# witalis3/UHSDR

Hardware: AMD Instinct MI355X
Metric: Msamples/s through full SSB-RX chain (node); % of HBM-roofline per GPU (higher is better)
Workload: dtype f32; 1 GPU; C2: 4096 ch x 256-frame blocks, SSB-USB P48 chain, f32; channels_per_gpu=4096, frames_per_call=256, parallelism=channel-sharded x1, no data-path collective, outputs=f32 audio, pipelined=True, handoff=persistent, precision=exact, schedule=split_pipe

## Files before the change

uhsdr_amd/csrc/uhsdr_dsp.h:

```cpp
#ifndef UHSDR_DSP_H
#define UHSDR_DSP_H

#include <hip/hip_runtime.h>
#include <stdint.h>
#include "uhsdr_internal.h"

#define BLK UHSDR_IQ_BLOCK_SIZE
#define IQ_BIT_SCALE_DOWN 0.0000152587890625f

typedef float vf4 __attribute__((ext_vector_type(4)));

template <int V, int N>
__device__ __forceinline__ void lds_vec(const float* p, float (&w)[N], int j)
{
    if (V == 4)
    {
        const float4 v = *(const float4*)p;
        w[j] = v.x; w[j + 1] = v.y; w[j + 2] = v.z; w[j + 3] = v.w;
    }
    else
    {
        const float2 v = *(const float2*)p;
        w[j] = v.x; w[j + 1] = v.y;
    }
// ... 107 lines not shown
        }
        else
        {
#pragma unroll
            for (int q = 0; q < 8; ++q) cc[q] = c[8 * ch + q];
        }
        v2f nw[8];
#pragma unroll
        for (int q = 0; q < 8; q += 2)
        {
            const vf4 v = *(const vf4*)(win + (16 + PB) * ch + pwin_off<PB>(WA + q));
            nw[q] = v.xy; nw[q + 1] = v.zw;
        }
#pragma unroll
        for (int kk = 0; kk < 8; ++kk)
        {
#pragma unroll
            for (int r = 0; r < R; ++r) acc[r] = fir_mac<F>(acc[r], w[r * M + kk], cc[kk]);
        }
#pragma unroll
        for (int j = 0; j < WA - 8; ++j) w[j] = w[j + 8];
#pragma unroll
        for (int q = 0; q < 8; ++q) w[WA - 8 + q] = nw[q];
    }
#pragma unroll
    for (int kk = 0; kk < TR; ++kk)
    {
        const v2f ck = TP ? cn[kk] : c[8 * NCH + kk];
#pragma unroll
        for (int r = 0; r < R; ++r) acc[r] = fir_mac<F>(acc[r], w[r * M + kk], ck);
    }
}

constexpr int FRONT_TAIL = 8;

__device__ __forceinline__ float to_vgpr(float x)
{
    float r;
    asm volatile("v_mov_b32 %0, %1" : "=v"(r) : "s"(x));
    return r;
}
template <int N>
__device__ __forceinline__ void to_vgpr(float (&x)[N])
{
#pragma unroll
    for (int i = 0; i < N; ++i) x[i] = to_vgpr(x[i]);
}

__device__ __forceinline__ void wave_sync()
{
    __builtin_amdgcn_fence(__ATOMIC_RELEASE, "wavefront");
    __builtin_amdgcn_wave_barrier();
    __builtin_amdgcn_fence(__ATOMIC_ACQUIRE, "wavefront");
}

__device__ __forceinline__ void lds_barrier()
{
    asm volatile("s_waitcnt lgkmcnt(0)" ::: "memory");
    __builtin_amdgcn_s_barrier();
    asm volatile("" ::: "memory");
}

constexpr int FRONT_WAVE = 64;
#define FRONT_WAVE_L 64

__host__ __device__ constexpr int hist_stride(int T) { return (T - 1 + 3) & ~3; }
__host__ __device__ constexpr int hist_q(int T) { return (hist_stride(T) / 4 + 7) / 8; }


template <int T, int HQM>
__device__ __forceinline__ void front_load_row(const float* row, int cl, int b, int nb, vf4 (&buf)[HQM])
{
    constexpr int hs4 = hist_stride(T) / 4, HQ = hist_q(T);
    const vf4* h = (const vf4*)(row + (size_t)cl * (hs4 * 4));
#pragma unroll
    for (int i = 0; i < HQ; ++i)
    {
        const int q = b + nb * i;
        buf[i] = h[q < hs4 ? q : hs4 - 1];
    }
}

template <int T, int HQM>
__device__ __forceinline__ void front_fill(float* W, float* row, int c, bool act, bool live, int b, int nb,
                                           const vf4 (&buf)[HQM], const float* vals, int NV)
{
// ... 234 lines not shown
        if (((T - 1 + b * NV) & 3) == 0 && (NV & 3) == 0)
            for (int j = 0; j < NV; j += 4) *(vf4*)(d + j) = vf4{ vals[j], vals[j + 1], vals[j + 2], vals[j + 3] };
        else if (((T - 1 + b * NV) & 1) == 0 && (NV & 1) == 0)
            for (int j = 0; j < NV; j += 2) *(v2f*)(d + j) = v2f{ vals[j], vals[j + 1] };
        else
            for (int j = 0; j < NV; ++j) d[j] = vals[j];
    }
}

__host__ __device__ inline void front_lane(int l, int nb, int S, int& g, int& b)
{
    const int cpw = 64 / nb, K = 64 / S, cpg = S / 4;
    if ((nb & (nb - 1)) || nb < K || cpw < cpg)
    {
        g = l / nb;
        b = l % nb;
        return;
    }
    const int h = l & 31;
    int k, j;
    if (h < 4) { k = 0; j = h; }
    else if (h < 12) { k = 1; j = h - 4; }
    else if (h < 16) { k = 0; j = h - 8; }
    else if (h < 20) { k = 1; j = h - 8; }
    else if (h < 28) { k = 0; j = h - 12; }
    else { k = 1; j = h - 16; }
    k += (l >> 5) * 2;
    const int pr = k * cpg + j / K;
    g = pr % cpw;
    b = (pr / cpw) * K + j % K;
}

template <int S>
__device__ __forceinline__ float lattice_step(float x, float (&g)[S > 0 ? S : 1], const float* k, const float* v)
{
    float fcurr = x, fnext = 0.0f, acc = 0.0f;
    float gn[S > 0 ? S : 1];
#pragma unroll
    for (int i = 0; i < S; ++i)
    {
        const float gcurr = g[i];
        fnext = fcurr - (k[i] * gcurr);
        const float gnext = (fnext * k[i]) + gcurr;
        acc += (gnext * v[i]);
        gn[i] = gnext;
        fcurr = fnext;
    }
    acc += (fnext * v[S]);
#pragma unroll
    for (int i = 0; i + 1 < S; ++i) g[i] = gn[i + 1];
    if (S > 0) g[S - 1] = fnext;
    return acc;
}

template <int S, int PAR>
__device__ __forceinline__ float lattice_step_pk(float x, float (&g)[S > 0 ? S : 1], const float* k, const float* v)
{
    if constexpr (S < 3) return lattice_step<S>(x, g, k, v);
    else
    {
        float gn[S], q[S];
        float f = x;
        int i = 0;
        if (PAR)
        {
            f = f - (k[0] * g[0]);
// ... 211 lines not shown
```

uhsdr_amd/csrc/uhsdr_rx.hip:

```cpp

#include <hip/hip_runtime.h>
#include <hip/hip_ext.h>
#include <stdint.h>
#include <string.h>
#include <stdlib.h>
#include <math.h>
#include <chrono>
#include "uhsdr_internal.h"
#include "uhsdr_libm.h"
#include "uhsdr_log10f_fast.h"
#include "uhsdr_dsp.h"

#define BACK_CH 64
constexpr int CNT_PITCH = 32;

struct FrontArgs
{
    const uhsdr_rx_plan* plan;
    const int2* iq;
    float* hist1;
    float* hist2;
    const uint16_t* lanemap;
    const uint16_t* lanemap2;
    int nb, cpw;
    float* teta;
    int* tp;
    unsigned* clip;
    const float* osc_in;
    float* osc_out;
    float* adec;
    float* adec_q;
    const float* taps2a;
    const float* taps2b;
    int C, N, ld, ldd;
    int lw;
    int comb;
    float* fm_prev;
    unsigned* gcnt;
};

enum { FRONT_COMB_USB = 0,
       FRONT_COMB_LSB = 1,
       FRONT_COMB_I = 2,
       FRONT_COMB_SSB_ST = 3,
       FRONT_COMB_IQ_ST = 4 };

template <int R>
__device__ __forceinline__ void front_comb_block(int comb, const v2f (&h)[R], float (&o)[R])
{
    if (comb == FRONT_COMB_I)
    {
#pragma unroll
        for (int r = 0; r < R; ++r) o[r] = h[r].x;
    }
    else if (comb == FRONT_COMB_LSB)
    {
#pragma unroll
        for (int r = 0; r < R; ++r) o[r] = h[r].x - h[r].y;
    }
    else
    {
#pragma unroll
        for (int r = 0; r < R; ++r) o[r] = h[r].x + h[r].y;
    }
}
__device__ __forceinline__ v2f front_comb2(int comb, v2f h)
{
    return comb == FRONT_COMB_SSB_ST ? v2f{ h.x + h.y, h.x - h.y } : h;
}

struct InputStage
// ... 90 lines not shown
    }
    if (!s.iq_auto)
    {
        if (s.gi != 1.0f || s.gq != 1.0f)
        {
#pragma unroll
            for (int j = 0; j < R; ++j) { xi[j] = xi[j] * s.gi; xq[j] = xq[j] * s.gq; }
        }
        if (s.ph < 0)
        {
#pragma unroll
            for (int j = 0; j < R; ++j) { const float e3 = xi[j] * s.ph; xq[j] = xq[j] + e3; }
        }
        else if (s.ph > 0)
        {
#pragma unroll
            for (int j = 0; j < R; ++j) { const float e3 = xq[j] * s.ph; xi[j] = xi[j] + e3; }
        }
    }
    else
    {
        const int bb = n0 / BLK;
        const float f1 = m1[bb], f2 = m2[bb];
#pragma unroll
        for (int j = 0; j < R; ++j) { xq[j] += f1 * xi[j]; xi[j] = xi[j] * f2; }
    }
    if (s.shift)
    {
        if (s.shift_up) freq_shift_block<R>(xi, xq, s.shift, osc, n0);
        else freq_shift_block<R>(xq, xi, s.shift, osc, n0);
    }
}

template <int T1, int T2, int M, bool DECIM_FIRST, int R, bool F, bool ST, typename Sink>
__device__ __forceinline__ void front_body(const FrontArgs& a, const int grp, float* smem, Sink&& sink)
{
    const uhsdr_rx_plan* __restrict__ P = a.plan;
    const int N = a.N, C = a.C;
    const int lane = threadIdx.x & (FRONT_WAVE - 1);
    const int nb = a.nb;
    const int CPW = a.cpw;
    const unsigned lm = a.lanemap[lane];
    const int g = (int)(lm >> 8), b = (int)(lm & 0xffu);
    const bool act = g < CPW;
    const int gs = act ? g : 0;
    const int nblk32 = N / BLK;
    constexpr int RD = R / M;
    constexpr int HQ1 = hist_qp(T1), HQ2 = hist_q(T2 > 0 ? T2 : 1), HQP2 = hist_qp(T2 > 0 ? T2 : 1);
    const int LW = a.lw;
    constexpr int PB1 = front_pad1(R, DECIM_FIRST, M);
    float* W = smem + gs * LW;
    float* aux = smem + CPW * LW;
    float* m1 = aux;
    float* m2 = aux + CPW * nblk32;
    float* osc = aux + (P->iq_auto_correction ? 2 * CPW * nblk32 : 0);
    float* fmx = osc + ((P->freq_shift_hz != 0 && P->shift_kind == 2) ? 2 * N : 0);

    InputStage in;
    in.gi = P->iq_gain_i; in.gq = P->iq_gain_q; in.ph = P->iq_phase_balance;
    in.iq_auto = P->iq_auto_correction;
    in.shift = P->freq_shift_hz != 0 ? P->shift_kind : 0;
    in.shift_up = P->shift_up;
    ctaps2_t* tA = as_taps2(a.taps2a);
    const int comb = a.comb;

    int4 raw[R / 2];
    vf4 hA[HQ1];
    const int c = grp * CPW + g;
    const bool live = act && c < C;
    const int cl = c < C ? c : C - 1;
    const int c0 = grp * CPW;
    const int nlive = C - c0 < CPW ? C - c0 : CPW;
    {
        const int4* src = (const int4*)(a.iq + (size_t)cl * a.ld + b * R);
#pragma unroll
        for (int j = 0; j < R / 2; ++j) raw[j] = src[j];
        group_load_prow<T1>(a.hist1, c0, nlive, lane, hA);
    }
    if (a.clip)
    {
        const unsigned f = clip_flags<R>(raw);
        if (f && live) atomicOr(a.clip + c, f);
    }
    if (in.shift == 2 && lane == 0)
    {
        const float oc = P->osc_cos, os = P->osc_sin;
        float vi = a.osc_in[0], vq = a.osc_in[1];
        for (int n = 0; n < N; ++n)
        {
            const float oq = (vq * oc) - (vi * os);
            const float oi = (vi * oc) + (vq * os);
            osc[2 * n] = oq;
            osc[2 * n + 1] = oi;
            vq = oq; vi = oi;
            if ((n & (BLK - 1)) == BLK - 1)
            {
                const float gn = (3 - ((vq * vq) + (vi * vi))) / 2;
                vq = gn * vq; vi = gn * vi;
            }
        }
        if (grp == 0) { a.osc_out[0] = vi; a.osc_out[1] = vq; }
    }

    {
        if (in.iq_auto)
        {
            for (int e = lane; e < CPW * nblk32; e += FRONT_WAVE)
            {
                const int gg = e / nblk32, bb = e % nblk32;
                const int cc = grp * CPW + gg;
                float t1 = 0.0f, t2 = 0.0f, t3 = 0.0f;
                if (cc < C)
// ... 21 lines not shown
                int tst = a.tp[cc], tcnt = a.tp[C + cc], trst = a.tp[2 * C + cc], truns = a.tp[3 * C + cc];
                float tph = __int_as_float(a.tp[4 * C + cc]);
                for (int bb = 0; bb < nblk32; ++bb)
                {
                    const int e = gg * nblk32 + bb;
                    float t1 = m1[e], t2 = m2[e], t3 = smem[e];
                    t1 = (float)(-0.003 * (double)(t1 / (float)BLK) + 0.997 * (double)o1);
                    t2 = (float)(0.003 * (double)(t2 / (float)BLK) + 0.997 * (double)o2);
                    t3 = (float)(0.003 * (double)(t3 / (float)BLK) + 0.997 * (double)o3);
                    const float M_c1 = (t2 != 0.0f) ? t1 / t2 : 0.0f;
                    float help = (t2 * t2);
                    if (help > 0.0f) help = (t3 * t3 - t1 * t1) / help;
                    const float M_c2 = (help > 0.0f) ? sqrtf(help) : 1.0f;
                    twinpeaks_step(t1, t3, tst, tcnt, trst, truns, tph);
                    m1[e] = M_c1;
                    m2[e] = M_c2;
                    o1 = t1; o2 = t2; o3 = t3;
                }
                a.teta[cc] = o1; a.teta[C + cc] = o2; a.teta[2 * C + cc] = o3;
                a.tp[cc] = tst; a.tp[C + cc] = tcnt; a.tp[2 * C + cc] = trst; a.tp[3 * C + cc] = truns;
                a.tp[4 * C + cc] = __float_as_int(tph);
            }
        }
        wave_sync();

        v2f x2[R];
        {
            float xi[R], xq[R];
            convert_block<R>(raw, in, b * R, m1 + gs * nblk32, m2 + gs * nblk32, osc, xi, xq);
#pragma unroll
            for (int j = 0; j < R; ++j) x2[j] = v2f{ xi[j], xq[j] };
        }
        group_fill_prow<T1, PB1>(smem, LW, a.hist1, c0, CPW, nlive, lane, hA);
        wave_sync();
        window_new2<PB1>(W, T1, act, b, x2, R);
        wave_sync();
        group_store_prow<T1, PB1>(smem, LW, a.hist1, c0, nlive, lane, nb * R);

        const unsigned lm2 = T2 ? a.lanemap2[lane] : lm;
        const int g2 = (int)(lm2 >> 8), b2 = (int)(lm2 & 0xffu);
        const bool act2 = g2 < CPW;
        const int c2 = grp * CPW + g2;
        const bool live2 = act2 && c2 < C;
        float* const W2 = smem + (act2 ? g2 : 0) * LW;
        float o[RD];
        if constexpr (T2 == 0)
        {
                v2f d2[RD];
            fir_block2<T1, RD, M, F, PB1>(W + pwin_off<PB1>(b * R), tA, d2);
            if constexpr (M == 1)
            {
                const bool translate = P->freq_shift_hz != 0;
                if (act)
                {
                    fmx[2 * (g * nb + b)] = d2[RD - 1].x;
                    fmx[2 * (g * nb + b) + 1] = d2[RD - 1].y;
                }
                wave_sync();
                const int pb = 2 * (g * nb + (b > 0 ? b - 1 : 0));
                const float li = fmx[pb], lq = fmx[pb + 1];
                const float si = a.fm_prev[cl], sq = a.fm_prev[C + cl];
                float ip = b > 0 ? li : si, qp = b > 0 ? lq : sq;
#pragma unroll
                for (int r = 0; r < RD; ++r)
                {
                    const float xi = d2[r].x, xq = d2[r].y;
                    const float y = (ip * xq) - (xi * qp);
                    const float x = (ip * xi) + (xq * qp);
                    o[r] = translate ? ul_atan2f(y, x) : 0.0f;
                    ip = xi; qp = xq;
                }
                if (translate && live && b == nb - 1)
                {
                    a.fm_prev[c] = d2[RD - 1].x;
                    a.fm_prev[C + c] = d2[RD - 1].y;
                }
            }
            else
            {
#pragma unroll
                for (int r = 0; r < RD; ++r) o[r] = d2[r].x;
                if (live)
                {
                    float* dst = a.adec_q + (size_t)c * a.ldd + b * RD;
#pragma unroll
                    for (int r = 0; r < RD; ++r) dst[r] = d2[r].y;
                }
            }
        }
        else if constexpr (!DECIM_FIRST && ST)
        {
            vf4 hC[HQP2];
            group_load_prow<T2>(a.hist2, c0, nlive, lane, hC);
            v2f h2[R], d2[RD];
            fir_block2<T1, R, 1, F, PB1>(W + pwin_off<PB1>(b * R), tA, h2);
#pragma unroll
            for (int r = 0; r < R; ++r) h2[r] = front_comb2(comb, h2[r]);
            wave_sync();
            group_fill_prow<T2>(smem, LW, a.hist2, c0, CPW, nlive, lane, hC);
            wave_sync();
            window_new2(W, T2, act, b, h2, R);
            wave_sync();
            group_store_prow<T2>(smem, LW, a.hist2, c0, nlive, lane, nb * R);
            fir_block2<T2, RD, M, F>(W2 + 2 * b2 * R, as_taps2(a.taps2b), d2);
#pragma unroll
            for (int r = 0; r < RD; ++r) o[r] = d2[r].x;
            if (live2)
            {
                float* dst = a.adec_q + (size_t)c2 * a.ldd + b2 * RD;
#pragma unroll
                for (int r = 0; r < RD; ++r) dst[r] = d2[r].y;
            }
        }
        else if constexpr (!DECIM_FIRST)
        {
            vf4 hC[HQ2];
            group_load_rows<T2>(a.hist2, c0, nlive, lane, hC);
            v2f h2[R];
            float hs[R];
            fir_block2<T1, R, 1, F, PB1>(W + pwin_off<PB1>(b * R), tA, h2);
            front_comb_block<R>(comb, h2, hs);
            wave_sync();
            group_fill_rows<T2>(smem, LW, a.hist2, c0, CPW, nlive, lane, hC);
            wave_sync();
            window_new(W, T2, act, b, hs, R);
            wave_sync();
            group_store_rows<T2>(smem, LW, a.hist2, c0, nlive, lane, nb * R);
            fir_block<T2, RD, M, 4, F>(W2 + b2 * R, as_taps(P->dec), o);
        }
        else
        {
            vf4 hC[HQP2];
            group_load_prow<T2>(a.hist2, c0, nlive, lane, hC);
            v2f d2[RD], h2[RD];
            fir_block2<T1, RD, M, F, PB1>(W + pwin_off<PB1>(b * R), tA, d2);
            wave_sync();
            group_fill_prow<T2>(smem, LW, a.hist2, c0, CPW, nlive, lane, hC);
            wave_sync();
            window_new2(W, T2, act, b, d2, RD);
            wave_sync();
            group_store_prow<T2>(smem, LW, a.hist2, c0, nlive, lane, nb * RD);
            fir_block2<T2, RD, 1, F>(W2 + 2 * b2 * RD, as_taps2(a.taps2b), h2);
            if constexpr (ST)
            {
#pragma unroll
                for (int r = 0; r < RD; ++r)
                {
                    const v2f st2 = front_comb2(comb, h2[r]);
                    o[r] = st2.x;
                    h2[r].y = st2.y;
                }
                if (live2)
                {
                    float* dst = a.adec_q + (size_t)c2 * a.ldd + b2 * RD;
#pragma unroll
                    for (int r = 0; r < RD; ++r) dst[r] = h2[r].y;
                }
            }
            else
            {
                front_comb_block<RD>(comb, h2, o);
            }
        }
        sink(live2, c2, g2, b2, o);
    }
}

template <int T1, int T2, int M, bool DECIM_FIRST, int R, bool F, bool ST = false>
__global__ void __launch_bounds__(FRONT_WAVE) rx_front(FrontArgs a)
{
    extern __shared__ __attribute__((aligned(16))) float smem[];
    constexpr int RD = R / M;
    front_body<T1, T2, M, DECIM_FIRST, R, F, ST>(a, blockIdx.x, smem,
        [&](bool live, int c, int, int b, const float (&o)[RD])
        {
            if (!live) return;
            float* dst = a.adec + (size_t)c * a.ldd + b * RD;
            if (a.gcnt)
            {
#pragma unroll
                for (int r = 0; r < RD; ++r) __hip_atomic_store(dst + r, o[r], __ATOMIC_RELAXED, __HIP_MEMORY_SCOPE_AGENT);
            }
            else if (RD % 4 == 0)
            {
#pragma unroll
                for (int r = 0; r < RD; r += 4) *(float4*)(dst + r) = make_float4(o[r], o[r + 1], o[r + 2], o[r + 3]);
            }
            else
            {
#pragma unroll
                for (int r = 0; r < RD; ++r) dst[r] = o[r];
            }
        });
    if (a.gcnt)
    {
        asm volatile("s_waitcnt vmcnt(0)" ::: "memory");
        if ((threadIdx.x & (FRONT_WAVE - 1)) == 0)
        {
            const int c0 = blockIdx.x * a.cpw;
            const int c1 = (c0 + a.cpw < a.C ? c0 + a.cpw : a.C) - 1;
            __hip_atomic_fetch_add(a.gcnt + (c0 / BACK_CH) * CNT_PITCH, 1u, __ATOMIC_RELAXED, __HIP_MEMORY_SCOPE_AGENT);
            if (c1 / BACK_CH != c0 / BACK_CH)
                __hip_atomic_fetch_add(a.gcnt + (c1 / BACK_CH) * CNT_PITCH, 1u, __ATOMIC_RELAXED, __HIP_MEMORY_SCOPE_AGENT);
        }
    }
}


constexpr int AGC_Q = 6;

struct BackState
{
    float* pre;
    float* aa;
    float* bq1;
    float* bq2;
    float* interp;
    float* ring;
    float* ring1;
    float* agc;
    int* agci;
    float* sam;
    float* cw;
    float *pre1, *aa1, *bq1_1, *bq2_1, *interp1;
    float* notch;
};

struct BackArgs
{
    const uhsdr_rx_plan* plan;
    const float* adec;
    const float* adec_q;
    float* audio;
    float* audio0;
    int2* dst;
    BackState s;
// ... 1927 lines not shown
            au.end(a, l, call);
        }
        if constexpr (TAP) nr_rows_store(a, l, call0, gc, xs, a.tap);
        else wave_sync();
    }
    au.store(a, l);
    aa.store(l, a.s.aa);
    ou.store(a, l);
}

template <int AA, int L, int PH, bool TAP = false>
__global__ void __launch_bounds__(BACK_CH) rx_nr_tail(BackArgs a, const float* row)
{
    static_assert(L == 4, "the firmware runs the stage on its 12 ksps paths only");
    __shared__ float xs[BACK_CH * FUSED_YPITCH];
    __shared__ float ys[BACK_CH * FUSED_YPITCH];
    if (a.plan->cw_enabled) nr_tail_body<AA, L, PH, true, TAP>(a, row, xs, ys);
    else nr_tail_body<AA, L, PH, false, TAP>(a, row, xs, ys);
}

template <int T1, int T2, int M, bool DF, int R, bool F, int PRE, int AA, int L, int PH, int W, bool TAP = false>
__global__ void __launch_bounds__(FRONT_WAVE) __attribute__((amdgpu_waves_per_eu(FUSED_WAVES)))
rx_chain(FrontArgs fa, BackArgs ba, int front_floats)
{
    static_assert(M == L, "decimation and interpolation rates agree");
    extern __shared__ __attribute__((aligned(16))) float smem[];
    constexpr int RD = R / M;
    float* adl = smem + front_floats;
    const int nb = fa.N / R, cpw = FRONT_WAVE / nb, passes = BACK_CH / cpw;
    const int grp = blockIdx.x;
    for (int p = 0; p < passes; ++p)
    {
        if ((grp * passes + p) * cpw >= fa.C) break;
        front_body<T1, T2, M, DF, R, F, false>(fa, grp * passes + p, smem,
            [&](bool, int, int g, int b, const float (&o)[RD])
            {
                float* d = adl + p * cpw + g;
#pragma unroll
                for (int r = 0; r < RD; ++r) d[(b * RD + r) * CHAIN_ADP] = o[r];
            });
        wave_sync();
    }
    if constexpr (TAP)
    {
        if (ba.plan->cw_enabled) back_fused_agc<PRE, AA, L, PH, W, DM_NONE, true, true, false, true>(ba, smem, grp, adl);
        else back_fused_agc<PRE, AA, L, PH, W, DM_NONE, false, true, false, true>(ba, smem, grp, adl);
        return;
    }
    if constexpr (L == 4)
    {
        if (ba.plan->cw_enabled) { back_fused_agc<PRE, AA, L, PH, W, DM_NONE, true, true, false>(ba, smem, grp, adl); return; }
    }
    back_fused_agc<PRE, AA, L, PH, W, DM_NONE, false, true, false>(ba, smem, grp, adl);
}

template <int PRE, int AA, int L, int PH, int W, int DM>
__global__ void __launch_bounds__(BACK_CH) rx_back_stereo(BackArgs a)
{
    const BackLane l(a);
    constexpr int NDC = BLK / L;
    static_assert(L == 2 || L == 4, "4 output frames per 1 or 2 decimated samples");
    const uhsdr_rx_plan* __restrict__ P = a.plan;
    const uhsdr_agc_plan A = P->agc;
    BackArgs b = a;
    b.adec = a.adec_q;
    b.s.bq1 = a.s.bq1_1; b.s.bq2 = a.s.bq2_1; b.s.interp = a.s.interp1;
    DemodStage<L, DM> dm;
// ... 342 lines not shown
        const float lo = P->line_out_scale, fs = P->fm_scale;
        for (int it = 0; it <= calls; ++it)
        {
            if (it > 0)
            {
                const int call = it - 1;
                const float* mi = dem + (call & 1) * BLK * BACK_CH + lane;
                const bool on = act[(call & 1) * BACK_CH + lane] != 0.0f;
#pragma unroll 2
                for (int n0 = 0; n0 < BLK; n0 += 4)
                {
                    float v[4];
#pragma unroll
                    for (int j = 0; j < 4; ++j)
                        v[j] = biquad_step(mi[(n0 + j) * BACK_CH] * fs, bq2[0], bq2[1], bq2[2], bq2[3], b2) * lo;
                    if (live) line_out4(a, (size_t)c * a.N + call * BLK + n0, 0u, call, call * BLK + n0, v, on);
                }
            }
            lds_barrier();
        }
        if (live)
        {
#pragma unroll
            for (int i = 0; i < 4; ++i) a.s.bq2[i * C + c] = bq2[i];
        }
    }
}


typedef void (*front_fn)(FrontArgs);
typedef void (*back_fn)(BackArgs);

typedef void (*chain_fn)(FrontArgs, BackArgs, int);
struct FrontVariant { int t1, t2, m, decim_first; front_fn fn; int R; front_fn fn_fma; int st; };
struct BackVariant { int pre, aa, L, ph, w, dm; back_fn fn; back_fn fused; back_fn fused_nodc; back_fn fused_ssb; back_fn fn_pers;
                     back_fn fn_tap; back_fn fused_tap; };
template <int PRE, int AA, int L, int PH, int W, int DM>
constexpr back_fn tap_of()
{
    if constexpr (DM == DM_NONE && L == 4) return rx_back<PRE, AA, L, PH, W, DM, false, true>;
    else return nullptr;
}
template <int PRE, int AA, int L, int PH, int W, int DM>
constexpr back_fn fused_tap_of()
{
    if constexpr (DM == DM_NONE && L == 4) return rx_back_fused<PRE, AA, L, PH, W, DM, false, 2>;
    else return nullptr;
}
template <int PRE, int AA, int L, int PH, int W, int DM>
constexpr back_fn pers_of()
{
    if constexpr (DM == DM_NONE) return rx_back<PRE, AA, L, PH, W, DM, true>;
    else return nullptr;
}
template <int PRE, int AA, int L, int PH, int W, int DM>
constexpr back_fn fused_nodc_of()
{
    if constexpr (DM == DM_NONE) return rx_back_fused<PRE, AA, L, PH, W, DM, false>;
    else return rx_back_fused<PRE, AA, L, PH, W, DM>;
}
template <int PRE, int AA, int L, int PH, int W, int DM>
constexpr back_fn fused_ssb_of()
{
    if constexpr (DM == DM_NONE) return rx_back_fused<PRE, AA, L, PH, W, DM, false, 1>;
    else return nullptr;
}
struct ChainVariant { int t1, t2, m, decim_first, R, pre, aa, L, ph, w; chain_fn fn, fn_fma, fn_tap, fn_tap_fma; };
template <int T1, int T2, int M, bool DF, bool F, int PRE, int AA, int PH, int W>
constexpr chain_fn chain_tap_of()
{
    if constexpr (M == 4) return rx_chain<T1, T2, M, DF, 8, F, PRE, AA, M, PH, W, true>;
    else return nullptr;
}
#define CHAIN_V(t1, t2, m, df, pre, aa, ph, w) { t1, t2, m, df, 8, pre, aa, m, ph, w, \
    rx_chain<t1, t2, m, df, 8, false, pre, aa, m, ph, w>, rx_chain<t1, t2, m, df, 8, true, pre, aa, m, ph, w>, \
    chain_tap_of<t1, t2, m, df, false, pre, aa, ph, w>(), chain_tap_of<t1, t2, m, df, true, pre, aa, ph, w>() }

#define FRONT_V(t1, t2, m, df, R) { t1, t2, m, df, rx_front<t1, t2, m, df, R, false>, R, rx_front<t1, t2, m, df, R, true>, 0 }
#define FRONT_ST(t1, t2, m, df, R) { t1, t2, m, df, rx_front<t1, t2, m, df, R, false, true>, R, rx_front<t1, t2, m, df, R, true, true>, 1 }
struct NotchVariant { int L, dm; back_fn fn; };
typedef void (*nr_head_fn)(BackArgs, float*);
typedef void (*nr_tail_fn)(BackArgs, const float*);
struct NrStageVariant { int pre, aa, L, ph, w; nr_head_fn head; nr_tail_fn tail, tail_tap; };
#define NR_V(pre, aa, ph, w) { pre, aa, 4, ph, w, rx_nr_head<pre, 4, w>, rx_nr_tail<aa, 4, ph>, rx_nr_tail<aa, 4, ph, true> }
#include <uhsdr_rx_variants.inc>
#undef CHAIN_V
#undef NR_V

static int plan_dm(const uhsdr_rx_plan& p)
{
    if (p.dmod_mode == UHSDR_DEMOD_FM) return DM_FM;
    if (p.dmod_mode == UHSDR_DEMOD_AM) return DM_AM;
    if (p.dmod_mode == UHSDR_DEMOD_SAM)
        return p.sam_sideband == UHSDR_SAM_SIDEBAND_BOTH ? DM_SAM : p.stereo == 3 ? DM_SAM_ST : DM_SAM_SB;
    return DM_NONE;
}

static int front_frames(int N, int R) { return N < FRONT_WAVE * R ? N : FRONT_WAVE * R; }

static const FrontVariant* find_front(const uhsdr_rx_plan& p, int N = 0, int want = 8, bool strict = false)
{
    const int t1 = p.use_decimated_iq ? p.dec_taps : p.hilbert_taps;
    const int t2 = p.use_decimated_iq ? p.hilbert_taps : p.dec_taps;
    const int st = p.stereo == 1 || p.stereo == 2;
    const FrontVariant* best = nullptr;
    for (const FrontVariant& v : kFront)
        if (v.t1 == t1 && v.t2 == t2 && v.m == p.decimation_rate && v.decim_first == p.use_decimated_iq && v.st == st)
        {
            if (N && (N % v.R || front_frames(N, v.R) / v.R < 4)) continue;
            if (strict && v.R != want) continue;
            if (!best || (v.R == want && best->R != want)) best = &v;
// ... 42 lines not shown
        return nullptr;
    }
    for (const BackVariant& v : kBack)
        if (v.pre == p.pre_stages && v.aa == p.aa_stages && v.L == p.interp_L && v.ph == p.interp_phase &&
            v.w == p.agc.attack_buffsize && v.dm == dm)
            return &v;
    return nullptr;
}


constexpr int TAPS2_MAX = (UHSDR_MAX_FIR_TAPS + 7) & ~7;
constexpr int BACK_FUSED_MIN_CHANNELS = 131072;

constexpr int PIPE_GROUP = 4;
constexpr int PIPE_BUFS = 2 * PIPE_GROUP;

struct uhsdr_rx_s
{
    uhsdr_rx_plan plan;
    uhsdr_rx_plan* d_plan;
    const FrontVariant* fv;
    const BackVariant* bv;
    const NotchVariant* nv;
    const ChainVariant* cv;
    int C, N, Nd, Nf;
    int lw;
    int schedule;
    int precision;
    int T1, T2;
    hipStream_t stream;
    float *hist1, *hist2, *teta, *osc, *adec, *adec_q;
    uint16_t* d_lanemap;
    uint16_t lmap[2][2][64];
    int* tp;
    unsigned* clip;
    float* d_taps2;
    BackState bs;
    void* arena;
    size_t arena_bytes;
    long long dec_samples;
    int cw_count;
    int cw_bmax, cw_blocks_last;
    int beep_left;
    uint32_t beep_acc;
    uint8_t* cw_signal;
    float* cw_energy;
    uhsdr_cwdec_handle cwt;
    uint8_t* cwt_signal;
    float* tap;
    uhsdr_rtty_handle rtty;
    uhsdr_psk_handle psk;
    float* text_tap;
    const NrStageVariant* nsv;
    uhsdr_nr_handle nr;
    float *nr_in, *nr_out;
    long long calls_done;
    long long front_launches;
    int pipelined;
    hipStream_t side;
    hipEvent_t ev_front, ev_join, ev_back[2];
    hipEvent_t ev_switch;
    float *adecp[PIPE_BUFS - 1], *adec_qp[PIPE_BUFS - 1];
    long long calls_issued;
    long long pipe_calls;
    int side_dirty;
    struct
// ... 157 lines not shown
        dst[2 * k + 1] = k < T ? c1[k] : 0.0f;
    }
}

static size_t front_lds_extra(const uhsdr_rx_s* h)
{
    const int N = h->Nf;
    const int cpw = FRONT_WAVE / (N / h->fv->R);
    size_t f = 0;
    if (h->plan.iq_auto_correction) f += 2 * cpw * (N / BLK);
    if (h->plan.freq_shift_hz != 0 && h->plan.shift_kind == 2) f += 2 * N;
    if (h->fv->m == 1) f += 2 * FRONT_WAVE;
    return f;
}

static size_t front_lds(const uhsdr_rx_s* h)
{
    const int N = h->Nf;
    const int cpw = FRONT_WAVE / (N / h->fv->R);
    size_t f = (size_t)cpw * h->lw + front_lds_extra(h) + FRONT_SLACK;
    return f * sizeof(float);
}

static size_t chain_front_floats(const uhsdr_rx_s* h)
{
    const size_t f = front_lds(h) / sizeof(float), ys = (size_t)BACK_CH * FUSED_YPITCH;
    return ((f > ys ? f : ys) + 3) & ~(size_t)3;
}
static size_t chain_lds(const uhsdr_rx_s* h)
{
    return sizeof(float) * (chain_front_floats(h) + (size_t)h->Nd * CHAIN_ADP);
}

static uhsdr_status configure_front(uhsdr_rx_s* h, int R, bool strict)
{
    const FrontVariant* fv = find_front(h->plan, h->N, R, strict);
    if (!fv) { uhsdr_set_error("no front kernel with %d outputs per lane for %d-frame calls", R, h->N); return UHSDR_UNSUPPORTED; }
    const FrontVariant* old = h->fv;
    const int oNf = h->Nf, olw = h->lw;
    h->fv = fv;
    h->T1 = fv->t1; h->T2 = fv->t2;
    h->Nf = front_frames(h->N, fv->R);
    uint16_t lm[2][64];
    h->lw = front_window_pitch(h, lm[0], lm[1]);
    uhsdr_status st = UHSDR_OK;
    if (h->N % h->Nf) { uhsdr_set_error("frames_per_call %d not a multiple of %d", h->N, h->Nf); st = UHSDR_LENGTH_ERROR; }
    else if (front_lds(h) > 64 * 1024) { uhsdr_set_error("frames_per_call too long for LDS"); st = UHSDR_LENGTH_ERROR; }
    if (st != UHSDR_OK && old) { h->fv = old; h->T1 = old->t1; h->T2 = old->t2; h->Nf = oNf; h->lw = olw; }
    if (st == UHSDR_OK)
    {
        const int k = fv->R == 16 ? 1 : 0;
        memcpy(h->lmap[k], lm, sizeof lm);
        if (h->d_lanemap && hipMemcpy(h->d_lanemap + 128 * k, lm, sizeof lm, hipMemcpyHostToDevice) != hipSuccess)
        {
            uhsdr_set_error("lane map upload failed");
            st = UHSDR_DEVICE_ERROR;
        }
    }
    return st;
}

static bool chain_ok(const uhsdr_rx_s* h)
{
    return h->cv && h->fv->R == h->cv->R && h->Nf == h->N && BACK_CH % (FRONT_WAVE / (h->Nf / h->fv->R)) == 0 &&
           chain_lds(h) <= 64 * 1024 && !h->plan.agc.remove_dc;
}

static size_t back_lds(const uhsdr_rx_s* h);

static int resolve_schedule(const uhsdr_rx_s* h, int want)
{
    if (want == UHSDR_SCHEDULE_AUTO)
    {
        if (h->C < BACK_FUSED_MIN_CHANNELS) return UHSDR_SCHEDULE_SPLIT_PIPE;
        return h->bv->fused ? UHSDR_SCHEDULE_SPLIT_FUSED : UHSDR_SCHEDULE_SPLIT_PIPE;
    }
    if (want == UHSDR_SCHEDULE_CHAIN) return chain_ok(h) ? want : -1;
    if (want == UHSDR_SCHEDULE_SPLIT_FUSED) return h->bv->fused ? want : -1;
    if (want == UHSDR_SCHEDULE_SPLIT_PIPE) return want;
    return -1;
}

static back_fn fused_back_fn(const uhsdr_rx_s* h)
{
    const BackVariant* bv = h->bv;
// ... 549 lines not shown
}

static int front_comb_of(const uhsdr_rx_plan& p)
{
    if (p.stereo == 1) return FRONT_COMB_SSB_ST;
    if (p.stereo == 2) return FRONT_COMB_IQ_ST;
    if (p.dmod_mode == UHSDR_DEMOD_IQ) return FRONT_COMB_I;
    return p.lsb ? FRONT_COMB_LSB : FRONT_COMB_USB;
}

static FrontArgs front_args(const uhsdr_rx_s* h, const int32_t* iq, int f0, float* adec, float* adec_q)
{
    FrontArgs fa;
    fa.plan = h->d_plan;
    fa.iq = (const int2*)iq + f0;
    fa.hist1 = h->hist1; fa.hist2 = h->hist2;
    fa.nb = h->Nf / h->fv->R;
    fa.cpw = FRONT_WAVE / fa.nb;
    fa.lanemap = h->d_lanemap + (h->fv->R == 16 ? 128 : 0);
    fa.lanemap2 = fa.lanemap + 64;
    fa.teta = h->teta;
    fa.tp = h->tp;
    fa.clip = h->clip;
    fa.osc_in = h->osc + 2 * (h->front_launches & 1);
    fa.osc_out = h->osc + 2 * ((h->front_launches + 1) & 1);
    fa.adec = adec ? adec + f0 / h->plan.decimation_rate : nullptr;
    fa.adec_q = adec_q ? adec_q + f0 / h->plan.decimation_rate : nullptr;
    fa.C = h->C; fa.N = h->Nf; fa.ld = h->N; fa.ldd = h->Nd;
    fa.lw = h->lw;
    fa.taps2a = h->d_taps2;
    fa.taps2b = h->d_taps2 + 2 * TAPS2_MAX;
    fa.comb = front_comb_of(h->plan);
    fa.gcnt = nullptr;
    fa.fm_prev = h->bs.sam;
    return fa;
}

static BackArgs back_args(uhsdr_rx_s* h, float* adec, float* adec_q, float* audio, float* audio0, int32_t* dst)
{
    BackArgs ba;
    ba.plan = h->d_plan;
    ba.adec = adec;
    ba.adec_q = adec_q;
    ba.audio = audio;
    ba.audio0 = h->plan.stereo || h->plan.single_channel ? audio0 : nullptr;
    ba.mchf = h->plan.single_channel != 0;
    ba.dst = (int2*)dst;
    ba.s = h->bs;
    ba.C = h->C; ba.N = h->N; ba.Nd = h->Nd;
    ba.ring_phase = (int)(h->calls_done % (h->bv->dm == DM_FM ? 200 : AGC_Q));
    ba.cw_signal = h->bs.cw ? (h->cw_signal || !h->cwt ? h->cw_signal : h->cwt_signal) : nullptr;
    ba.cw_energy = h->bs.cw ? h->cw_energy : nullptr;
    ba.cw_count0 = h->cw_count;
    ba.cw_bmax = h->cw_bmax;
    ba.tap = tap_row(h);
    {
        const int slots = NOTCH_DELAY / (BLK / h->plan.decimation_rate);
        ba.notch_slot0 = (int)(h->calls_done % slots);
        ba.notch_first = h->calls_done == 0;
    }
    ba.tone_phase = (int)(h->calls_done % 400);
    ba.dwait = nullptr;
    ba.dtarget = 0;
    ba.spin_max = h->spin_max;
    ba.fail = h->fail_dev;
    ba.adec_next = nullptr;
// ... 134 lines not shown
        }
        if (done()) return UHSDR_OK;
    }
}

static uhsdr_status wait_release(uhsdr_rx_s* h, const RxRoute& r)
{
    if (r.pm)
    {
        const unsigned* pw = h->run.pmem;
        const unsigned need = r.seq - (PIPE_BUFS - 1);
        return pers_spin([&]() {
            for (int g = 0; g < r.bgroups; ++g)
                if ((int)(__atomic_load_n(pw + PC_CONSUMED + g, __ATOMIC_ACQUIRE) - need) < 0) return false;
            return true;
        }, "persistent back end: call %u's hand-off buffer not released within 30 s", r.seq);
    }
    if (r.side && r.pk % PIPE_GROUP == 0) HIPCHK(hipStreamWaitEvent(h->stream, h->ev_back[r.grp], 0));
    return UHSDR_OK;
}

static uhsdr_status launch_fronts(uhsdr_rx_s* h, const RxRoute& r, const int32_t* iq, bool fma)
{
    const size_t lds = front_lds(h);
    time_mark(h, K_FRONT, 0);
    for (int f0 = 0; f0 < h->N; f0 += h->Nf)
    {
        FrontArgs fa = front_args(h, iq, f0, r.adec, r.adec_q);
        if (r.dfl)
        {
            fa.gcnt = r.gc;
            h->hand.fills[r.par] += 1;
        }
        const auto fn = fma ? h->fv->fn_fma : h->fv->fn;
        const dim3 grid((h->C + r.cpw - 1) / r.cpw), block(FRONT_WAVE);
        if (r.side && !r.dfl && f0 + h->Nf >= h->N)
            hipExtLaunchKernelGGL(fn, grid, block, lds, h->stream, nullptr, h->ev_front, 0, fa);
        else
            hipLaunchKernelGGL(fn, grid, block, lds, h->stream, fa);
        HIPCHK(hipGetLastError());
        h->front_launches += 1;
    }
    time_mark(h, K_FRONT, 1);
    return UHSDR_OK;
}

static void handoff_args(const uhsdr_rx_s* h, const RxRoute& r, BackArgs& bk)
{
    bk.dwait = r.gc;
    bk.dtarget = h->hand.fills[r.par];
    bk.fcpw = r.cpw;
    if (h->hand.skew && h->N / BLK >= BACK_SKEW && !h->bs.cw && !bk.tap)
    {
        const int parn = (int)((r.pk + 1) % PIPE_BUFS);
        bk.adec_next = parn ? h->adecp[parn - 1] : h->adec;
        bk.dwait_next = h->hand.gcnt + (size_t)parn * r.bgroups * CNT_PITCH;
        bk.dnext = h->hand.fills[parn] + (unsigned)((h->N + h->Nf - 1) / h->Nf);
    }
}

static uhsdr_status pers_grant(uhsdr_rx_s* h, const RxRoute& r, BackArgs& bk, bool& launch)
{
    unsigned* const pw = h->run.pmem;
    const unsigned seq = r.seq;
    BackDesc* d = (BackDesc*)(pw + PC_WORDS) + seq % DESC_RING;
    d->adec = r.adec;
    d->cnt = r.gc;
// ... 458 lines not shown
```

Before: 56040 Msamples/s.

## Add lean front-end kernel variant with computed lane maps and packed stores

Adds a LEAN specialization of the front kernel. It computes lane-to-channel mappings arithmetically instead of loading them, and drops clip detection, IQ auto-correction and the shift_kind 2 oscillator paths. It also skips the bounds checks and writes hand-off outputs as 64-bit atomic stores. A packed-math FIR decimator (fir_block_pm) and explicit vector-memory drains before the wave syncs are added as well. The host selects the lean kernel only when the persistent hand-off is used and the lane maps, alignment and plan flags match, which adds more template instantiations and host-side map checks.

```diff
diff --git a/uhsdr_amd/csrc/uhsdr_dsp.h b/uhsdr_amd/csrc/uhsdr_dsp.h
--- a/uhsdr_amd/csrc/uhsdr_dsp.h
+++ b/uhsdr_amd/csrc/uhsdr_dsp.h
@@ -163,6 +163,75 @@
     }
 }
 
+template <int T, int R, int M, bool F = false>
+__device__ __forceinline__ void fir_block_pm(const float* win, const float* taps, float (&acc)[R])
+{
+    if constexpr (F || R < 2 || (M & 1)) fir_block<T, R, M, 4, F>(win, as_taps(taps), acc);
+    else
+    {
+        ctaps_t* c = as_taps(taps);
+        constexpr int WA = (M * (R - 1) + 8 + 7) & ~7;
+        constexpr int NCH = T / 8, TR = T % 8;
+        static_assert(NCH <= 8, "fully unrolled: decimators only");
+        v2f w[WA / 2];
+#pragma unroll
+        for (int r = 0; r < R; ++r) acc[r] = 0.0f;
+#pragma unroll
+        for (int j = 0; j < WA; j += 4)
+        {
+            const vf4 v = *(const vf4*)(win + j);
+            w[j / 2] = v.xy; w[j / 2 + 1] = v.zw;
+        }
+#pragma unroll
+        for (int ch = 0; ch < NCH; ++ch)
+        {
+            v2f cc[4];
+#pragma unroll
+            for (int q = 0; q < 4; ++q) cc[q] = v2f{ c[8 * ch + 2 * q], c[8 * ch + 2 * q + 1] };
+            v2f nw[4];
+#pragma unroll
+            for (int q = 0; q < 8; q += 4)
+            {
+                const vf4 v = *(const vf4*)(win + 8 * ch + WA + q);
+                nw[q / 2] = v.xy; nw[q / 2 + 1] = v.zw;
+            }
+#pragma unroll
+            for (int kk = 0; kk < 8; kk += 2)
+            {
+#pragma unroll
+                for (int r = 0; r < R; ++r)
+                {
+                    const v2f p = w[(r * M + kk) / 2] * cc[kk / 2];
+                    acc[r] = acc[r] + p.x;
+                    acc[r] = acc[r] + p.y;
+                }
+            }
+#pragma unroll
+            for (int j = 0; j < WA / 2 - 4; ++j) w[j] = w[j + 4];
+#pragma unroll
+            for (int q = 0; q < 4; ++q) w[WA / 2 - 4 + q] = nw[q];
+        }
+#pragma unroll
+        for (int kk = 0; kk + 1 < TR; kk += 2)
+        {
+            const v2f ck = v2f{ c[8 * NCH + kk], c[8 * NCH + kk + 1] };
+#pragma unroll
+            for (int r = 0; r < R; ++r)
+            {
+                const v2f p = w[(r * M + kk) / 2] * ck;
+                acc[r] = acc[r] + p.x;
+                acc[r] = acc[r] + p.y;
+            }
+        }
+        if constexpr (TR & 1)
+        {
+            const float ck = c[8 * NCH + TR - 1];
+#pragma unroll
+            for (int r = 0; r < R; ++r) acc[r] = acc[r] + w[(r * M + TR - 1) / 2].x * ck;
+        }
+    }
+}
+
 constexpr int FRONT_TAIL = 8;
 
 __device__ __forceinline__ float to_vgpr(float x)
@@ -183,6 +252,11 @@
     __builtin_amdgcn_fence(__ATOMIC_RELEASE, "wavefront");
     __builtin_amdgcn_wave_barrier();
     __builtin_amdgcn_fence(__ATOMIC_ACQUIRE, "wavefront");
+}
+
+__device__ __forceinline__ void vmem_drain()
+{
+    __builtin_amdgcn_s_waitcnt(0x0f70);
 }
 
 __device__ __forceinline__ void lds_barrier()
@@ -483,6 +557,31 @@
 }
 
 template <int S>
+__host__ __device__ inline void front_lane_pow2(int l, int lnb, bool interleaved, int& g, int& b)
+{
+    const int nb = 1 << lnb, cpw = 64 >> lnb;
+    if (interleaved)
+    {
+        g = (l & 3) + 4 * (l >> (lnb + 2));
+        b = (l & (4 * nb - 1)) >> 2;
+        return;
+    }
+    constexpr int K = 64 / S, cpg = S / 4;
+    if (nb < K || cpw < cpg)
+    {
+        g = l >> lnb;
+        b = l & (nb - 1);
+        return;
+    }
+    const int h = l & 31;
+    const int k = ((h >= 4 && h < 12) || (h >= 16 && h < 20) || h >= 28 ? 1 : 0) + (l >> 5) * 2;
+    const int j = h < 4 ? h : h < 12 ? h - 4 : h < 20 ? h - 8 : h < 28 ? h - 12 : h - 16;
+    const int pr = k * cpg + j / K;
+    g = pr & (cpw - 1);
+    b = (pr >> (6 - lnb)) * K + (j & (K - 1));
+}
+
+template <int S>
 __device__ __forceinline__ float lattice_step(float x, float (&g)[S > 0 ? S : 1], const float* k, const float* v)
 {
     float fcurr = x, fnext = 0.0f, acc = 0.0f;
diff --git a/uhsdr_amd/csrc/uhsdr_rx.hip b/uhsdr_amd/csrc/uhsdr_rx.hip
--- a/uhsdr_amd/csrc/uhsdr_rx.hip
+++ b/uhsdr_amd/csrc/uhsdr_rx.hip
@@ -37,6 +37,7 @@
     int comb;
     float* fm_prev;
     unsigned* gcnt;
+    int lnb, mk1, mk2;
 };
 
 enum { FRONT_COMB_USB = 0,
@@ -193,20 +194,34 @@
     }
 }
 
-template <int T1, int T2, int M, bool DECIM_FIRST, int R, bool F, bool ST, typename Sink>
+template <int T1, int T2, int M, bool DECIM_FIRST, int R, bool F, bool ST, bool LEAN, typename Sink>
 __device__ __forceinline__ void front_body(const FrontArgs& a, const int grp, float* smem, Sink&& sink)
 {
     const uhsdr_rx_plan* __restrict__ P = a.plan;
     const int N = a.N, C = a.C;
     const int lane = threadIdx.x & (FRONT_WAVE - 1);
-    const int nb = a.nb;
-    const int CPW = a.cpw;
-    const unsigned lm = a.lanemap[lane];
-    const int g = (int)(lm >> 8), b = (int)(lm & 0xffu);
-    const bool act = g < CPW;
+    const int nb = LEAN ? 1 << a.lnb : a.nb;
+    const int CPW = LEAN ? FRONT_WAVE >> a.lnb : a.cpw;
+    constexpr int RD = R / M;
+    constexpr int S1 = 2 * R, S2 = (DECIM_FIRST || ST ? 2 : 1) * (DECIM_FIRST ? RD : R);
+    int g, b, g2, b2;
+    if constexpr (LEAN)
+    {
+        if (a.mk1 == 1) front_lane_pow2<S2>(lane, a.lnb, false, g, b);
+        else front_lane_pow2<S1>(lane, a.lnb, a.mk1 == 2, g, b);
+        if (a.mk2 == 1) front_lane_pow2<S2>(lane, a.lnb, false, g2, b2);
+        else front_lane_pow2<S1>(lane, a.lnb, a.mk2 == 2, g2, b2);
+    }
+    else
+    {
+        const unsigned lm = a.lanemap[lane];
+        const unsigned lm2 = T2 ? a.lanemap2[lane] : lm;
+        g = (int)(lm >> 8); b = (int)(lm & 0xffu);
+        g2 = (int)(lm2 >> 8); b2 = (int)(lm2 & 0xffu);
+    }
+    const bool act = LEAN || g < CPW;
     const int gs = act ? g : 0;
     const int nblk32 = N / BLK;
-    constexpr int RD = R / M;
     constexpr int HQ1 = hist_qp(T1), HQ2 = hist_q(T2 > 0 ? T2 : 1), HQP2 = hist_qp(T2 > 0 ? T2 : 1);
     const int LW = a.lw;
     constexpr int PB1 = front_pad1(R, DECIM_FIRST, M);
@@ -219,8 +234,8 @@
 
     InputStage in;
     in.gi = P->iq_gain_i; in.gq = P->iq_gain_q; in.ph = P->iq_phase_balance;
-    in.iq_auto = P->iq_auto_correction;
-    in.shift = P->freq_shift_hz != 0 ? P->shift_kind : 0;
+    in.iq_auto = LEAN ? 0 : P->iq_auto_correction;
+    in.shift = P->freq_shift_hz != 0 ? (LEAN ? 1 : P->shift_kind) : 0;
     in.shift_up = P->shift_up;
     ctaps2_t* tA = as_taps2(a.taps2a);
     const int comb = a.comb;
@@ -228,17 +243,17 @@
     int4 raw[R / 2];
     vf4 hA[HQ1];
     const int c = grp * CPW + g;
-    const bool live = act && c < C;
-    const int cl = c < C ? c : C - 1;
+    const bool live = LEAN || (act && c < C);
+    const int cl = LEAN || c < C ? c : C - 1;
     const int c0 = grp * CPW;
-    const int nlive = C - c0 < CPW ? C - c0 : CPW;
+    const int nlive = LEAN || C - c0 >= CPW ? CPW : C - c0;
     {
         const int4* src = (const int4*)(a.iq + (size_t)cl * a.ld + b * R);
 #pragma unroll
         for (int j = 0; j < R / 2; ++j) raw[j] = src[j];
         group_load_prow<T1>(a.hist1, c0, nlive, lane, hA);
     }
-    if (a.clip)
+    if (!LEAN && a.clip)
     {
         const unsigned f = clip_flags<R>(raw);
         if (f && live) atomicOr(a.clip + c, f);
@@ -326,16 +341,15 @@
             for (int j = 0; j < R; ++j) x2[j] = v2f{ xi[j], xq[j] };
         }
         group_fill_prow<T1, PB1>(smem, LW, a.hist1, c0, CPW, nlive, lane, hA);
+        vmem_drain();
         wave_sync();
         window_new2<PB1>(W, T1, act, b, x2, R);
         wave_sync();
         group_store_prow<T1, PB1>(smem, LW, a.hist1, c0, nlive, lane, nb * R);
 
-        const unsigned lm2 = T2 ? a.lanemap2[lane] : lm;
-        const int g2 = (int)(lm2 >> 8), b2 = (int)(lm2 & 0xffu);
-        const bool act2 = g2 < CPW;
+        const bool act2 = LEAN || g2 < CPW;
         const int c2 = grp * CPW + g2;
-        const bool live2 = act2 && c2 < C;
+        const bool live2 = LEAN || (act2 && c2 < C);
         float* const W2 = smem + (act2 ? g2 : 0) * LW;
         float o[RD];
         if constexpr (T2 == 0)
@@ -392,6 +406,7 @@
             for (int r = 0; r < R; ++r) h2[r] = front_comb2(comb, h2[r]);
             wave_sync();
             group_fill_prow<T2>(smem, LW, a.hist2, c0, CPW, nlive, lane, hC);
+            vmem_drain();
             wave_sync();
             window_new2(W, T2, act, b, h2, R);
             wave_sync();
@@ -416,11 +431,12 @@
             front_comb_block<R>(comb, h2, hs);
             wave_sync();
             group_fill_rows<T2>(smem, LW, a.hist2, c0, CPW, nlive, lane, hC);
+            vmem_drain();
             wave_sync();
             window_new(W, T2, act, b, hs, R);
             wave_sync();
             group_store_rows<T2>(smem, LW, a.hist2, c0, nlive, lane, nb * R);
-            fir_block<T2, RD, M, 4, F>(W2 + b2 * R, as_taps(P->dec), o);
+            fir_block_pm<T2, RD, M, F>(W2 + b2 * R, P->dec, o);
         }
         else
         {
@@ -430,6 +446,7 @@
             fir_block2<T1, RD, M, F, PB1>(W + pwin_off<PB1>(b * R), tA, d2);
             wave_sync();
             group_fill_prow<T2>(smem, LW, a.hist2, c0, CPW, nlive, lane, hC);
+            vmem_drain();
             wave_sync();
             window_new2(W, T2, act, b, d2, RD);
             wave_sync();
@@ -460,20 +477,41 @@
     }
 }
 
-template <int T1, int T2, int M, bool DECIM_FIRST, int R, bool F, bool ST = false>
+template <int RD, bool WIDE>
+__device__ __forceinline__ void handoff_store(float* dst, const float (&o)[RD])
+{
+    if constexpr (WIDE && RD % 2 == 0)
+    {
+#pragma unroll
+        for (int r = 0; r < RD; r += 2)
+        {
+            const unsigned long long v = (unsigned long long)__float_as_uint(o[r]) | (unsigned long long)__float_as_uint(o[r + 1]) << 32;
+            __hip_atomic_store((unsigned long long*)(dst + r), v, __ATOMIC_RELAXED, __HIP_MEMORY_SCOPE_AGENT);
+        }
+    }
+    else
+    {
+#pragma unroll
+        for (int r = 0; r < RD; ++r) __hip_atomic_store(dst + r, o[r], __ATOMIC_RELAXED, __HIP_MEMORY_SCOPE_AGENT);
+    }
+}
+
+template <int T1, int T2, int M, bool DECIM_FIRST, int R, bool F, bool ST = false, bool LEAN = false>
 __global__ void __launch_bounds__(FRONT_WAVE) rx_front(FrontArgs a)
 {
     extern __shared__ __attribute__((aligned(16))) float smem[];
     constexpr int RD = R / M;
-    front_body<T1, T2, M, DECIM_FIRST, R, F, ST>(a, blockIdx.x, smem,
+    const bool wide = LEAN || (RD % 2 == 0 && (((uintptr_t)a.adec | ((uintptr_t)a.ldd << 2)) & 7) == 0);
+    front_body<T1, T2, M, DECIM_FIRST, R, F, ST, LEAN>(a, blockIdx.x, smem,
         [&](bool live, int c, int, int b, const float (&o)[RD])
         {
             if (!live) return;
             float* dst = a.adec + (size_t)c * a.ldd + b * RD;
-            if (a.gcnt)
-            {
-#pragma unroll
-                for (int r = 0; r < RD; ++r) __hip_atomic_store(dst + r, o[r], __ATOMIC_RELAXED, __HIP_MEMORY_SCOPE_AGENT);
+            if constexpr (LEAN) handoff_store<RD, true>(dst, o);
+            else if (a.gcnt)
+            {
+                if (wide) handoff_store<RD, true>(dst, o);
+                else handoff_store<RD, false>(dst, o);
             }
             else if (RD % 4 == 0)
             {
@@ -486,16 +524,20 @@
                 for (int r = 0; r < RD; ++r) dst[r] = o[r];
             }
         });
-    if (a.gcnt)
+    if (LEAN || a.gcnt)
     {
         asm volatile("s_waitcnt vmcnt(0)" ::: "memory");
         if ((threadIdx.x & (FRONT_WAVE - 1)) == 0)
         {
-            const int c0 = blockIdx.x * a.cpw;
-            const int c1 = (c0 + a.cpw < a.C ? c0 + a.cpw : a.C) - 1;
+            const int cpw = LEAN ? FRONT_WAVE >> a.lnb : a.cpw;
+            const int c0 = blockIdx.x * cpw;
             __hip_atomic_fetch_add(a.gcnt + (c0 / BACK_CH) * CNT_PITCH, 1u, __ATOMIC_RELAXED, __HIP_MEMORY_SCOPE_AGENT);
-            if (c1 / BACK_CH != c0 / BACK_CH)
-                __hip_atomic_fetch_add(a.gcnt + (c1 / BACK_CH) * CNT_PITCH, 1u, __ATOMIC_RELAXED, __HIP_MEMORY_SCOPE_AGENT);
+            if constexpr (!LEAN)
+            {
+                const int c1 = (c0 + cpw < a.C ? c0 + cpw : a.C) - 1;
+                if (c1 / BACK_CH != c0 / BACK_CH)
+                    __hip_atomic_fetch_add(a.gcnt + (c1 / BACK_CH) * CNT_PITCH, 1u, __ATOMIC_RELAXED, __HIP_MEMORY_SCOPE_AGENT);
+            }
         }
     }
 }
@@ -2489,7 +2531,7 @@
     for (int p = 0; p < passes; ++p)
     {
         if ((grp * passes + p) * cpw >= fa.C) break;
-        front_body<T1, T2, M, DF, R, F, false>(fa, grp * passes + p, smem,
+        front_body<T1, T2, M, DF, R, F, false, false>(fa, grp * passes + p, smem,
             [&](bool, int, int g, int b, const float (&o)[RD])
             {
                 float* d = adl + p * cpw + g;
@@ -2898,7 +2940,13 @@
 typedef void (*back_fn)(BackArgs);
 
 typedef void (*chain_fn)(FrontArgs, BackArgs, int);
-struct FrontVariant { int t1, t2, m, decim_first; front_fn fn; int R; front_fn fn_fma; int st; };
+struct FrontVariant { int t1, t2, m, decim_first; front_fn fn; int R; front_fn fn_fma; int st; front_fn fn_lean, fn_lean_fma; };
+template <int T1, int T2, int M, bool DF, int R, bool F>
+constexpr front_fn front_lean_of()
+{
+    if constexpr (T2 != 0) return rx_front<T1, T2, M, DF, R, F, false, true>;
+    else return nullptr;
+}
 struct BackVariant { int pre, aa, L, ph, w, dm; back_fn fn; back_fn fused; back_fn fused_nodc; back_fn fused_ssb; back_fn fn_pers;
                      back_fn fn_tap; back_fn fused_tap; };
 template <int PRE, int AA, int L, int PH, int W, int DM>
@@ -2942,7 +2990,8 @@
     rx_chain<t1, t2, m, df, 8, false, pre, aa, m, ph, w>, rx_chain<t1, t2, m, df, 8, true, pre, aa, m, ph, w>, \
     chain_tap_of<t1, t2, m, df, false, pre, aa, ph, w>(), chain_tap_of<t1, t2, m, df, true, pre, aa, ph, w>() }
 
-#define FRONT_V(t1, t2, m, df, R) { t1, t2, m, df, rx_front<t1, t2, m, df, R, false>, R, rx_front<t1, t2, m, df, R, true>, 0 }
+#define FRONT_V(t1, t2, m, df, R) { t1, t2, m, df, rx_front<t1, t2, m, df, R, false>, R, rx_front<t1, t2, m, df, R, true>, 0, \
+    front_lean_of<t1, t2, m, df, R, false>(), front_lean_of<t1, t2, m, df, R, true>() }
 #define FRONT_ST(t1, t2, m, df, R) { t1, t2, m, df, rx_front<t1, t2, m, df, R, false, true>, R, rx_front<t1, t2, m, df, R, true, true>, 1 }
 struct NotchVariant { int L, dm; back_fn fn; };
 typedef void (*nr_head_fn)(BackArgs, float*);
@@ -3051,6 +3100,7 @@
     float *hist1, *hist2, *teta, *osc, *adec, *adec_q;
     uint16_t* d_lanemap;
     uint16_t lmap[2][2][64];
+    int lean_lnb, lean_mk[2];
     int* tp;
     unsigned* clip;
     float* d_taps2;
@@ -3274,6 +3324,47 @@
     return sizeof(float) * (chain_front_floats(h) + (size_t)h->Nd * CHAIN_ADP);
 }
 
+static bool front_lane_pow2_rt(int S, int l, int lnb, bool interleaved, int& g, int& b)
+{
+    switch (S)
+    {
+    case 4: front_lane_pow2<4>(l, lnb, interleaved, g, b); return true;
+    case 8: front_lane_pow2<8>(l, lnb, interleaved, g, b); return true;
+    case 16: front_lane_pow2<16>(l, lnb, interleaved, g, b); return true;
+    case 32: front_lane_pow2<32>(l, lnb, interleaved, g, b); return true;
+    default: return false;
+    }
+}
+
+static void front_lean_maps(uhsdr_rx_s* h, const uint16_t (&lm)[2][64])
+{
+    const int R = h->fv->R, nb = h->Nf / R;
+    h->lean_lnb = -1;
+    if (nb < 4 || nb > 64 || (nb & (nb - 1))) return;
+    int lnb = 0;
+    while ((1 << lnb) < nb) ++lnb;
+    const bool df = h->fv->decim_first != 0;
+    const int RD = R / h->fv->m;
+    const int S[2] = { 2 * R, (df || h->fv->st ? 2 : 1) * (df ? RD : R) };
+    for (int pass = 0; pass < 2; ++pass)
+    {
+        int kind = -1;
+        for (int k = 0; k < 3 && kind < 0; ++k)
+        {
+            bool same = true;
+            for (int l = 0; l < 64 && same; ++l)
+            {
+                int g = 0, b = 0;
+                same = front_lane_pow2_rt(S[k == 1], l, lnb, k == 2, g, b) && lm[pass][l] == (uint16_t)(g << 8 | b);
+            }
+            if (same) kind = k;
+        }
+        if (kind < 0) return;
+        h->lean_mk[pass] = kind;
+    }
+    h->lean_lnb = lnb;
+}
+
 static uhsdr_status configure_front(uhsdr_rx_s* h, int R, bool strict)
 {
     const FrontVariant* fv = find_front(h->plan, h->N, R, strict);
@@ -3293,6 +3384,7 @@
     {
         const int k = fv->R == 16 ? 1 : 0;
         memcpy(h->lmap[k], lm, sizeof lm);
+        front_lean_maps(h, lm);
         if (h->d_lanemap && hipMemcpy(h->d_lanemap + 128 * k, lm, sizeof lm, hipMemcpyHostToDevice) != hipSuccess)
         {
             uhsdr_set_error("lane map upload failed");
@@ -3908,6 +4000,7 @@
     fa.taps2b = h->d_taps2 + 2 * TAPS2_MAX;
     fa.comb = front_comb_of(h->plan);
     fa.gcnt = nullptr;
+    fa.lnb = h->lean_lnb; fa.mk1 = h->lean_mk[0]; fa.mk2 = h->lean_mk[1];
     fa.fm_prev = h->bs.sam;
     return fa;
 }
@@ -4108,7 +4201,12 @@
             fa.gcnt = r.gc;
             h->hand.fills[r.par] += 1;
         }
-        const auto fn = fma ? h->fv->fn_fma : h->fv->fn;
+        const uhsdr_rx_plan& p = h->plan;
+        const bool lean = r.dfl && h->fv->fn_lean && h->lean_lnb >= 0 && r.cpw == FRONT_WAVE >> h->lean_lnb &&
+                          h->C % r.cpw == 0 && !h->clip && !p.iq_auto_correction &&
+                          !(p.freq_shift_hz != 0 && p.shift_kind == 2) &&
+                          (((uintptr_t)fa.adec | ((uintptr_t)fa.ldd << 2)) & 7) == 0;
+        const auto fn = lean ? (fma ? h->fv->fn_lean_fma : h->fv->fn_lean) : fma ? h->fv->fn_fma : h->fv->fn;
         const dim3 grid((h->C + r.cpw - 1) / r.cpw), block(FRONT_WAVE);
         if (r.side && !r.dfl && f0 + h->Nf >= h->N)
             hipExtLaunchKernelGGL(fn, grid, block, lds, h->stream, nullptr, h->ev_front, 0, fa);
```

Result: slower. 54860 Msamples/s (-2.1%).
